# grant-froelich/Bathymetric-GNN

Measured on AMD Instinct MI355X. Metric: classified tile-nodes/s (fused graph build + 4-layer GAT forward + scatter), higher is better.
Workload: dtype f32

## Files before the change

### bathymetric-gnn_amd/csrc/bgnn_api.hip

```cpp
#include <stdarg.h>
#include <string.h>
#include <stdlib.h>

#include <algorithm>
#include <cmath>

#include "bgnn_internal.h"

namespace bgnn {

static thread_local char g_err[1024] = "";

void set_error(const char *fmt, ...) {
  va_list ap;
  va_start(ap, fmt);
  vsnprintf(g_err, sizeof(g_err), fmt, ap);
  va_end(ap);
}

int DevPool::alloc(size_t bytes, void **out) {
  if (bytes == 0) bytes = 256;
  bytes = (bytes + 255) & ~(size_t)255;
  auto it = free_blocks.lower_bound(bytes);
  if (it != free_blocks.end() && it->first <= bytes + bytes / 4 + 4096) {
// ... 177 lines not shown
}

using namespace bgnn;

extern "C" {

int bgnn_abi_version(void) { return BGNN_ABI_VERSION; }
const char *bgnn_last_error(void) { return g_err; }

int bgnn_ctx_create(int device, void *stream, bgnn_ctx **out) {
  BGNN_REQUIRE(out != nullptr, "bgnn_ctx_create: out is NULL");
  int n = 0;
  hipError_t e = hipGetDeviceCount(&n);
  if (e != hipSuccess || n <= 0) {
    (void)hipGetLastError();
    set_error("no HIP device available (%s)", e == hipSuccess ? "device count is 0" : hipGetErrorString(e));
    return BGNN_ERR_HIP;
  }
  BGNN_REQUIRE(device >= 0 && device < n, "bgnn_ctx_create: device %d out of range (have %d)", device, n);
  BGNN_HIP_CHECK(hipSetDevice(device));
  hipDeviceProp_t prop;
  BGNN_HIP_CHECK(hipGetDeviceProperties(&prop, device));
  bgnn_ctx *c = new bgnn_ctx();
  c->device = device;
  c->num_cus = prop.multiProcessorCount;
  if (stream) {
    c->stream = (hipStream_t)stream;
    c->owns_stream = false;
  } else {
    hipError_t se = hipStreamCreateWithFlags(&c->stream, hipStreamNonBlocking);
    if (se != hipSuccess) {
      delete c;
      set_error("hipStreamCreate failed: %s", hipGetErrorString(se));
      return BGNN_ERR_HIP;
    }
    c->owns_stream = true;
  }
  if (hipMalloc((void **)&c->zero_page, 16384) != hipSuccess || hipMemset(c->zero_page, 0, 16384) != hipSuccess) {
    set_error("zero page allocation failed");
    delete c;
    return BGNN_ERR_NOMEM;
  }
  c->stamps = reinterpret_cast<unsigned long long *>(c->zero_page + 1024);
  {
    auto env_int = [](const char *name, int dflt) { const char *e = getenv(name); return e ? atoi(e) : dflt; };
    BgnnOpts &o = c->opts;
    o.matrix_path = getenv("BGNN_BF16") ? 3 : getenv("BGNN_SPLIT_F16") ? 2 : getenv("BGNN_SPLIT_BF16") ? 1 : 0;
    o.fused = getenv("BGNN_NO_FUSED") ? 0 : 1;
    o.fold_extractor = getenv("BGNN_NO_FOLD") ? 0 : 1;
    o.ragged_atlas = getenv("BGNN_NO_ATLAS") ? 0 : 1;
    o.fused_front = getenv("BGNN_NO_FUSED_FRONT") ? 0 : 1;
    o.bf16_two_phase = getenv("BGNN_NO_TWO_PHASE") ? 0 : env_int("BGNN_TWO_PHASE", 1);
    o.bf16_layer0_af = getenv("BGNN_NO_LAYER0_AF") ? 0 : 1;
    o.stats_narrow = env_int("BGNN_STATS_NARROW", -1);
    o.diag_mask = env_int("BGNN_FUSED_DBG", 0);
    o.diag_stamps = getenv("BGNN_FUSED_STAMPS") ? 1 : 0;
    o.gemm_diag = env_int("BGNN_GEMM_DBG", 0);
    o.gemm_pair_major = getenv("BGNN_NO_PAIR_MAJOR") ? 0 : 1;
  }
  *out = c;
  return BGNN_OK;
}

static int *option_slot(bgnn_ctx *ctx, const char *name) {
  BgnnOpts &o = ctx->opts;
  struct { const char *n; int *p; } tab[] = {
      {"matrix_path", &o.matrix_path}, {"fused", &o.fused}, {"fold_extractor", &o.fold_extractor}, {"ragged_atlas", &o.ragged_atlas}, {"features_tiled", &o.features_tiled}, {"fused_front", &o.fused_front}, {"bf16_two_phase", &o.bf16_two_phase}, {"bf16_layer0_af", &o.bf16_layer0_af}, {"stats_narrow", &o.stats_narrow},
      {"diag_mask", &o.diag_mask}, {"diag_stamps", &o.diag_stamps}, {"gemm_diag", &o.gemm_diag}, {"gemm_pair_major", &o.gemm_pair_major}};
  for (auto &t : tab) if (strcmp(t.n, name) == 0) return t.p;
  return nullptr;
}

int bgnn_ctx_set_option(bgnn_ctx *ctx, const char *name, int value) {
  BGNN_REQUIRE(ctx && name, "bgnn_ctx_set_option: NULL argument");
  int *p = option_slot(ctx, name);
  BGNN_REQUIRE(p, "bgnn_ctx_set_option: unknown option '%s'", name);
  if (p == &ctx->opts.matrix_path) BGNN_REQUIRE(value >= 0 && value <= 3, "matrix_path=%d (0 exact f32, 1 bf16x3, 2 fp16x3, 3 bf16 storage)", value);
  if ((p == &ctx->opts.diag_mask || p == &ctx->opts.diag_stamps || p == &ctx->opts.gemm_diag) && value != 0)
    BGNN_REQUIRE(BGNN_DIAG, "option '%s' needs the diagnostic build of the library (python __graft_entry__.py --diag)", name);
  *p = value;
  return BGNN_OK;
}

int bgnn_ctx_get_option(bgnn_ctx *ctx, const char *name, int *value) {
  BGNN_REQUIRE(ctx && name && value, "bgnn_ctx_get_option: NULL argument");
  int *p = option_slot(ctx, name);
  BGNN_REQUIRE(p, "bgnn_ctx_get_option: unknown option '%s'", name);
  *value = *p;
  return BGNN_OK;
}

int bgnn_debug_stamps(bgnn_ctx *ctx, unsigned long long *out32) {
  if (!ctx || !out32) return BGNN_ERR_INVALID;
  (void)hipStreamSynchronize(ctx->stream);
  if (hipMemcpy(out32, ctx->stamps, 512, hipMemcpyDeviceToHost) != hipSuccess) return BGNN_ERR_HIP;
  (void)hipMemset(ctx->stamps, 0, 512);
  return BGNN_OK;
}

static void graph_free(bgnn_graph *g);

int bgnn_ctx_destroy(bgnn_ctx *ctx) {
  if (!ctx) return BGNN_OK;
  (void)hipSetDevice(ctx->device);
  (void)hipStreamSynchronize(ctx->stream);
  while (!ctx->live_graphs.empty()) graph_free(*ctx->live_graphs.begin());
  for (auto &r : ctx->prof_records) { (void)hipEventDestroy(r.start); (void)hipEventDestroy(r.stop); }
  for (auto &e : ctx->event_pool) (void)hipEventDestroy(e);
  for (auto &st : ctx->staging) { (void)hipEventDestroy(st.ev); (void)hipHostFree(st.p); }
  for (int i = 0; i < 7; ++i) if (ctx->ws[i]) (void)hipFree(ctx->ws[i]);
  for (auto &e : ctx->table_cache) { (void)hipFree(e.d_tiles); (void)hipFree(e.d_items); }
  if (ctx->zero_page) (void)hipFree(ctx->zero_page);
  ctx->pool.trim();
  for (auto &kv : ctx->pool.live) (void)hipFree(kv.first);
  if (ctx->owns_stream) (void)hipStreamDestroy(ctx->stream);
  delete ctx;
  return BGNN_OK;
}

int bgnn_ctx_synchronize(bgnn_ctx *ctx) {
// ... 585 lines not shown
```

### bathymetric-gnn_amd/csrc/bgnn_internal.h

```cpp
#pragma once
#include <hip/hip_runtime.h>
#include <stdint.h>
#include <stdio.h>
#include <string>
#include <cstdlib>
#include <vector>
#include <map>
#include <set>
#include <atomic>

#include "../../include/bgnn.h"
#include "../../include/bgnn_train.h"

namespace bgnn {

void set_error(const char *fmt, ...);

#define BGNN_HIP_CHECK(expr)                                                          \
  do {                                                                                \
    hipError_t _e = (expr);                                                           \
    if (_e != hipSuccess) {                                                           \
      bgnn::set_error("%s failed: %s (%s:%d)", #expr, hipGetErrorString(_e), __FILE__, \
                      __LINE__);                                                      \
      return BGNN_ERR_HIP;                                                            \
// ... 4 lines not shown
  do {                                 \
    if (!(cond)) {                     \
      bgnn::set_error(__VA_ARGS__);    \
      return BGNN_ERR_INVALID;         \
    }                                  \
  } while (0)

#define BGNN_TRY(expr)          \
  do {                          \
    int _r = (expr);            \
    if (_r != BGNN_OK) return _r; \
  } while (0)

struct DevPool {
  std::multimap<size_t, void *> free_blocks;
  std::map<void *, size_t> live;
  size_t total_bytes = 0;
  int alloc(size_t bytes, void **out);
  void release(void *p);
  void trim();
};

struct ProfRecord {
  int kernel;
  hipEvent_t start, stop;
};

struct WeightLayout {
  size_t fe_W0, fe_b0, fe_W1, fe_b1;
  struct Layer { size_t W, as, ad, ae, We, bias, bn_w, bn_b, bn_mean, bn_var, W2, b1; };
  std::vector<Layer> layers;
  size_t hd_W0[3], hd_b0[3], hd_W1[3], hd_b1[3];
  size_t total;
};

}

struct BgnnTileMeta {
  int32_t h, w;
  int32_t cell_off;
  int32_t pad;
  double rx, ry;
};

struct BgnnWorkItem {
  int32_t tile, r0, nr, pad;
};

struct BgnnOpts {
  int matrix_path = 0;
  int fused = 1;
  int fold_extractor = 1;
  int bf16_two_phase = 1;
  int bf16_layer0_af = 1;
  int stats_narrow = -1;
  int fused_front = 1;
  int features_tiled = 1;
  int ragged_atlas = 1;
  int diag_mask = 0;
  int diag_stamps = 0;
  int gemm_diag = 0;
  int gemm_pair_major = 1;
};

#ifndef BGNN_DIAG
#define BGNN_DIAG 0
#endif

struct bgnn_ctx {
  int device = 0;
  BgnnOpts opts;
  hipStream_t stream = nullptr;
  bool owns_stream = false;
  bgnn::DevPool pool;
  uint32_t prof_mask = 0;
  std::vector<bgnn::ProfRecord> prof_records;
  std::vector<hipEvent_t> event_pool;
  void *ws[7] = {nullptr, nullptr, nullptr, nullptr, nullptr, nullptr, nullptr};
  size_t ws_bytes[7] = {0, 0, 0, 0, 0, 0, 0};
  struct Staging { void *p; size_t cap; hipEvent_t ev; bool in_flight; };
  std::vector<Staging> staging;
  struct TableCache { int32_t n_tiles, h, w, item_cells; double rx, ry; BgnnTileMeta *d_tiles; BgnnWorkItem *d_items; int32_t n_items; uint64_t stamp; uint64_t id; int32_t refs; };
  std::vector<TableCache> table_cache;
  uint64_t table_stamp = 0, table_next_id = 1;
  std::set<struct bgnn_graph *> live_graphs;
  int num_cus = 256;
  float *zero_page = nullptr;
  unsigned long long *stamps = nullptr;
};

struct BgnnLayer {
  int d_in, heads, width;
  int concat;
  float *Wt;
  float *Wt_blk = nullptr;
  float *att_src;
  float *att_dst;
  float *V;
  float *scale;
  float *shift;
  float *Wsp;
  float *Wsp16;
  float Wsp16_inv = 1.0f;
  float *Wfp;
  float *Wbf;
  float *b1;
// ... 221 lines not shown
```

### bathymetric-gnn_amd/csrc/gat_layer_fused.hip

```cpp
#include <stdlib.h>
#include <algorithm>
#include <type_traits>
#include <utility>
#include "gat_tile_common.h"

namespace bgnn {

typedef float f32x16 __attribute__((ext_vector_type(16)));

enum { EPI_NEXT = 0, EPI_HEADS = 1 };

#if BGNN_DIAG
#define DBG(bit) (a.dbg & (bit))
#define BGNN_STAMP(slot)                                                                   \
  if (a.stamps) {                                                                          \
    const unsigned long long _t = __builtin_amdgcn_s_memtime();                            \
    t_sum[slot] += _t - t_prev;                                                            \
    t_prev = _t;                                                                           \
  }
#else
#define DBG(bit) false
#define BGNN_STAMP(slot)
#endif

// ... 1565 lines not shown
      constexpr int NC4 = NC * 4;
      const int t = 2 * cp + tt;
      const f32x16 &acc = tt ? acc1 : acc0;
      f32x4 s4[4], d4[4];
      s4[0] = lds_read4<0>(asl + t * 128); s4[1] = lds_read4<32>(asl + t * 128);
      s4[2] = lds_read4<64>(asl + t * 128); s4[3] = lds_read4<96>(asl + t * 128);
      d4[0] = lds_read4<NC4>(asl + t * 128); d4[1] = lds_read4<NC4 + 32>(asl + t * 128);
      d4[2] = lds_read4<NC4 + 64>(asl + t * 128); d4[3] = lds_read4<NC4 + 96>(asl + t * 128);
      lds_reads_done();
#pragma unroll
      for (int g = 0; g < 4; ++g) {
        const float4 v = make_float4(acc[4 * g], acc[4 * g + 1], acc[4 * g + 2], acc[4 * g + 3]);
        const f32x2 vlo = {v.x, v.y}, vhi = {v.z, v.w};
        ps_ += vlo * (f32x2){s4[g].x, s4[g].y}; ps_ += vhi * (f32x2){s4[g].z, s4[g].w};
        pd_ += vlo * (f32x2){d4[g].x, d4[g].y}; pd_ += vhi * (f32x2){d4[g].z, d4[g].w};
        typedef __bf16 bf16x4 __attribute__((ext_vector_type(4)));
        bf16x4 o;
        o[0] = (__bf16)v.x; o[1] = (__bf16)v.y; o[2] = (__bf16)v.z; o[3] = (__bf16)v.w;
        char *pb = patch + r * 128 + ((hl ^ ((r >> 3) & 1)) << 3);
        *reinterpret_cast<bf16x4 *>(pb + (((tt * 4 + g) ^ (r & 7)) << 4)) = o;
      }
      asm volatile("" : "+v"(ps_), "+v"(pd_));
      __builtin_amdgcn_sched_barrier(0);
    }
    sl_[cp] = ps_.x + ps_.y; dl_[cp] = pd_.x + pd_.y;
#pragma unroll
    for (int k = 0; k < NSTORE; ++k) {
      const int row = (lane >> 3) + 8 * k;
      uint4 q = *reinterpret_cast<const uint4 *>(patch + row * 128 + (((lane & 7) ^ (row & 7)) << 4));
      if (k & 1) q = make_uint4(q.z, q.w, q.x, q.y);
      char *prow = (rid_[k] >= 0 ? reinterpret_cast<char *>(a.out) + (int64_t)rid_[k] * (NC * 2) : reinterpret_cast<char *>(a.dump)) + (lane & 7) * 16;
      *reinterpret_cast<uint4 *>(prow + cp * 128) = q;
    }
    __builtin_amdgcn_sched_barrier(0);
  };
  col_pass(std::integral_constant<int, 0>{}); col_pass(std::integral_constant<int, 1>{});
  col_pass(std::integral_constant<int, 2>{}); col_pass(std::integral_constant<int, 3>{});
  {
    float srow[H2], drow_[H2];
#pragma unroll
    for (int hd = 0; hd < H2; ++hd) {
      const float sl = sl_[hd], dl = dl_[hd];
      srow[hd] = sl + __shfl_xor(sl, 32);
      drow_[hd] = dl + __shfl_xor(dl, 32);
    }
    if (id >= 0 && hl == 0) {
      float *ao = a.asd_out + (int64_t)id * 2 * H2;
      *reinterpret_cast<float4 *>(ao) = make_float4(srow[0], srow[1], srow[2], srow[3]);
      *reinterpret_cast<float4 *>(ao + 4) = make_float4(drow_[0], drow_[1], drow_[2], drow_[3]);
    }
  }
}

template <int K, bool AF = false>
static int launch_two_phase(bgnn_ctx *ctx, const FusedArgs &a) {
  constexpr size_t lds_bytes = (size_t)TwoPhaseLds<K>::BYTES;
  static std::atomic<uint64_t> configured{0};
  auto kern = gat_layer_bf16_2p_kernel<K, AF>;
  if (!(configured.load(std::memory_order_relaxed) >> (ctx->device & 63) & 1)) {
    BGNN_HIP_CHECK(hipFuncSetAttribute(reinterpret_cast<const void *>(kern), hipFuncAttributeMaxDynamicSharedMemorySize, (int)lds_bytes));
    configured.fetch_or(1ull << (ctx->device & 63), std::memory_order_relaxed);
  }
  hipLaunchKernelGGL(kern, dim3(a.tb.n_blocks), dim3(256), lds_bytes, ctx->stream, a);
  BGNN_HIP_CHECK(hipGetLastError());
  return BGNN_OK;
}

template <int HC, int C, int K, int NT, int EPI, int SP = 0, int AGG = 0>
static int launch_inst(bgnn_ctx *ctx, const FusedArgs &a) {
  constexpr size_t lds_bytes = (size_t)FusedLds<HC, C, K, NT, EPI, SP>::FLOATS * 4;
  static_assert(lds_bytes <= 160 * 1024, "one workgroup fits the CU's LDS");
  static std::atomic<uint64_t> configured{0};
  auto kern = gat_layer_fused_kernel<HC, C, K, NT, EPI, SP, AGG>;
  if (!(configured.load(std::memory_order_relaxed) >> (ctx->device & 63) & 1)) {
    BGNN_HIP_CHECK(hipFuncSetAttribute(reinterpret_cast<const void *>(kern), hipFuncAttributeMaxDynamicSharedMemorySize, (int)lds_bytes));
    configured.fetch_or(1ull << (ctx->device & 63), std::memory_order_relaxed);
  }
  hipLaunchKernelGGL(kern, dim3(a.tb.n_blocks), dim3(256), lds_bytes, ctx->stream, a);
  BGNN_HIP_CHECK(hipGetLastError());
  return BGNN_OK;
}

template <int HC, int NT, int EPI>
static int launch_by_stencil(bgnn_ctx *ctx, const bgnn_graph *g, int sp, const FusedArgs &a) {
  switch (sp) {
    case 0:
      return g->K == 8 ? launch_inst<HC, 64, 8, NT, EPI, 0>(ctx, a) : g->K == 4 ? launch_inst<HC, 64, 4, NT, EPI, 0>(ctx, a)
                                                                                 : launch_inst<HC, 64, 16, NT, EPI, 0>(ctx, a);
    case 3:
      return g->K == 8 ? launch_inst<HC, 64, 8, NT, EPI, 3>(ctx, a) : g->K == 4 ? launch_inst<HC, 64, 4, NT, EPI, 3>(ctx, a)
                                                                                 : launch_inst<HC, 64, 16, NT, EPI, 3>(ctx, a);
    default: break;
  }
  if (g->K == 16) return BGNN_ERR_UNSUPPORTED;
  if (sp == 1) return g->K == 8 ? launch_inst<HC, 64, 8, NT, EPI, 1>(ctx, a) : launch_inst<HC, 64, 4, NT, EPI, 1>(ctx, a);
  return g->K == 8 ? launch_inst<HC, 64, 8, NT, EPI, 2>(ctx, a) : launch_inst<HC, 64, 4, NT, EPI, 2>(ctx, a);
}

static bool fused_supported(const bgnn_graph *g, int C) {
  return g->kind == 0 && (g->K == 4 || g->K == 8 || g->K == 16) && g->n_blocks3 > 0 && C == 64 && g->max_w <= 8192 && g->compact_edges;
}

static void fill_common(FusedArgs &a, const bgnn_graph *g, const BgnnLayer &L, const float *V3, const void *xw, const float *asd, int relu) {
  a.tb.tiles = g->d_tiles; a.tb.items2 = g->uni_h ? nullptr : g->d_items3;
  a.tb.bh = g->bh3; a.tb.bw = g->bw3; a.tb.n_blocks = g->n_blocks3;
  a.node_id = g->d_node_id; a.cell_map = nullptr; a.tile_of_cell = nullptr;
  if (g->d_atlas) {
    a.tb.tiles = g->d_atlas_tile; a.tb.items2 = nullptr;
    a.tb.bh = g->atlas_h / 8; a.tb.bw = g->atlas_w / 16; a.tb.n_blocks = a.tb.bh * a.tb.bw;
    a.node_id = g->d_atlas; a.cell_map = g->d_cell_of_node; a.tile_of_cell = g->d_atlas_tile_of;
  }
  a.xw = xw; a.asd = asd; a.V = V3 ? V3 : L.V; a.scale = L.scale; a.shift = L.shift;
  a.slope = g->d_slope; a.node_depth = g->d_node_depth; a.tile_dist = g->d_tile_dist;
  a.relu = relu; a.zero_page = g->ctx->zero_page; a.dump = g->ctx->zero_page + 2048;
  a.dbg = BGNN_DIAG ? g->ctx->opts.diag_mask : 0;
  a.stamps = BGNN_DIAG && g->ctx->opts.diag_stamps ? g->ctx->stamps : nullptr;
}

int launch_fused_layer_next(bgnn_ctx *ctx, const bgnn_graph *g, const BgnnLayer &L, const BgnnLayer &Ln, int C, const float *V3,
                            const void *xw, const float *asd, void *xw_next, float *asd_next) {
  if (!fused_supported(g, C) || (!g->edge_default && !V3)) return BGNN_ERR_UNSUPPORTED;
  const int HC = L.heads * C, NC = Ln.heads * C;
  if (Ln.d_in != HC) return BGNN_ERR_UNSUPPORTED;
  FusedArgs a{};
  fill_common(a, g, L, V3, xw, asd, L.concat ? 1 : 0);
  int split = ctx->opts.matrix_path;
  if (split == 2 && !Ln.Wsp16) split = 1;
  a.Wt = split == 3 ? Ln.Wbf : split == 2 ? Ln.Wsp16 : split == 1 ? Ln.Wsp : Ln.Wfp;
  a.w_inv = Ln.Wsp16_inv;
  a.att_src = Ln.att_src; a.att_dst = Ln.att_dst; a.out = xw_next; a.asd_out = asd_next;
  a.H2 = Ln.heads; a.C2 = C;
  ProfScope ps(ctx, BGNN_K_FUSED);
  const bool main_shape = (HC == 256 && NC == 256) || (HC == 256 && NC == 64);
  if (split == 3 && !main_shape) return BGNN_ERR_UNSUPPORTED;
  if ((split == 1 || split == 2) && (!main_shape || g->K == 16)) { split = 0; a.Wt = Ln.Wfp; }
  if (split == 3 && HC == 256 && NC == 256 && C == 64 && ctx->opts.bf16_two_phase)
    return g->K == 8 ? launch_two_phase<8>(ctx, a) : g->K == 4 ? launch_two_phase<4>(ctx, a) : launch_two_phase<16>(ctx, a);
#define BGNN_FUSED_CASE(hc, nt) if (HC == hc && NC == nt * 32) return launch_by_stencil<hc, nt, EPI_NEXT>(ctx, g, split, a);
  BGNN_FUSED_CASE(256, 8) BGNN_FUSED_CASE(256, 2)
#undef BGNN_FUSED_CASE
  if (g->K == 16) return BGNN_ERR_UNSUPPORTED;
#define BGNN_FUSED_CASE(hc, nt)                                                                         \
  if (HC == hc && NC == nt * 32)                                                                        \
    return g->K == 8 ? launch_inst<hc, 64, 8, nt, EPI_NEXT>(ctx, a) : launch_inst<hc, 64, 4, nt, EPI_NEXT>(ctx, a);
  BGNN_FUSED_CASE(128, 4) BGNN_FUSED_CASE(128, 2) BGNN_FUSED_CASE(64, 2)
#undef BGNN_FUSED_CASE
  return BGNN_ERR_UNSUPPORTED;
}

int launch_fused_layer0_af(bgnn_ctx *ctx, const bgnn_graph *g, const BgnnLayer &L, const BgnnLayer &Ln, int C, const float *V3,
                           const void *h1, const float *asd, const float *W0af, const float *shift_af, void *xw_next, float *asd_next) {
  if (!fused_supported(g, C) || (!g->edge_default && !V3) || !W0af || !shift_af) return BGNN_ERR_UNSUPPORTED;
  if (C != 64 || L.heads != 4 || Ln.heads != 4 || Ln.d_in != 256 || !Ln.Wbf) return BGNN_ERR_UNSUPPORTED;
  FusedArgs a{};
  fill_common(a, g, L, V3, h1, asd, L.concat ? 1 : 0);
  a.shift = shift_af;
  a.Wt = Ln.Wbf; a.W0af = W0af;
  a.att_src = Ln.att_src; a.att_dst = Ln.att_dst; a.out = xw_next; a.asd_out = asd_next;
  a.H2 = Ln.heads; a.C2 = C;
  ProfScope ps(ctx, BGNN_K_FUSED);
  return g->K == 8 ? launch_two_phase<8, true>(ctx, a) : g->K == 4 ? launch_two_phase<4, true>(ctx, a) : launch_two_phase<16, true>(ctx, a);
}

int launch_fused_plain_layer(bgnn_ctx *ctx, const bgnn_graph *g, int mode, int C, const float *x, const float *dinv, const float *Wfp,
                             const float *ones, const float *post_scale, const float *post_shift, int post_relu, float *out) {
  if (!fused_supported(g, C) || !Wfp || mode < 1 || mode > 3) return BGNN_ERR_UNSUPPORTED;
  FusedArgs a{};
  BgnnLayer L{};
  L.V = nullptr; L.scale = const_cast<float *>(ones); L.shift = ctx->zero_page;
  fill_common(a, g, L, nullptr, x, dinv, 0);
  a.Wt = Wfp; a.att_src = post_scale; a.att_dst = post_shift; a.out = out; a.asd_out = nullptr;
  a.H2 = 1; a.C2 = C; a.relu2 = post_relu; a.self_loops = g->include_self_loops;
  ProfScope ps(ctx, BGNN_K_FUSED);
#define BGNN_PLAIN_CASE(M, HCV)                                                                                   \
  if (mode == M)                                                                                                  \
    return g->K == 8 ? launch_inst<HCV, 64, 8, 2, EPI_NEXT, 0, M>(ctx, a) : g->K == 4 ? launch_inst<HCV, 64, 4, 2, EPI_NEXT, 0, M>(ctx, a) \
                                                                                       : launch_inst<HCV, 64, 16, 2, EPI_NEXT, 0, M>(ctx, a);
  BGNN_PLAIN_CASE(1, 64) BGNN_PLAIN_CASE(2, 128) BGNN_PLAIN_CASE(3, 64)
#undef BGNN_PLAIN_CASE
  return BGNN_ERR_UNSUPPORTED;
}

bool fused_heads_available(const bgnn_ctx *ctx, const bgnn_graph *g, const bgnn_model *m) {
  if (!ctx->opts.fused || m->desc.gnn_type != BGNN_GNN_GAT || m->layers.empty()) return false;
  const BgnnLayer &L = m->layers.back();
  return fused_supported(g, m->desc.hidden) && L.heads == 1 && m->desc.num_classes <= 4 && m->head_hidden_total == 96 && m->hd_tab &&
         (m->desc.predict_correction ? 3 : 2) * (m->desc.hidden / 2) <= 96;
}

int launch_fused_layer_heads(bgnn_ctx *ctx, const bgnn_graph *g, const bgnn_model *m, const BgnnLayer &L, int C, const float *V3,
// ... 23 lines not shown
```

### bathymetric-gnn_amd/csrc/gat_tile_common.h

```cpp
#pragma once
#include "bgnn_internal.h"

namespace bgnn {

template <int K> struct StencilOffsets;
template <> struct StencilOffsets<4> {
  static constexpr int dr[4] = {-1, 1, 0, 0};
  static constexpr int dc[4] = {0, 0, -1, 1};
};
template <> struct StencilOffsets<8> {
  static constexpr int dr[8] = {-1, -1, -1, 0, 0, 1, 1, 1};
  static constexpr int dc[8] = {-1, 0, 1, -1, 1, -1, 0, 1};
};

template <> struct StencilOffsets<16> {
  static constexpr int dr[16] = {-1, -1, -1, 0, 0, 1, 1, 1, -2, -2, -2, 0, 0, 2, 2, 2};
  static constexpr int dc[16] = {-1, 0, 1, -1, 1, -1, 0, 1, -2, 0, 2, -2, 2, -2, 0, 2};
};

constexpr int TILE_W = 16;
constexpr int HALO_W = TILE_W + 2;
constexpr int TILED_PITCH = 36;
constexpr int TILE_H = 16, HALO_ROWS = (TILE_H + 2) * HALO_W;

template <int K>
__device__ __forceinline__ int slot_halo_offset(int b) {
  if (b >= K) return 0;
  if (K == 8) {
    const int k = b < 4 ? b : b + 1;
    return (k / 3 - 1) * (TILE_W + 2) + (k % 3 - 1);
  }
  return b == 0 ? -(TILE_W + 2) : b == 1 ? (TILE_W + 2) : b == 2 ? -1 : 1;
}

struct TileBlocks {
  const BgnnTileMeta *tiles;
  const BgnnWorkItem *items2;
  int bh, bw;
  int n_blocks;
};

struct BlockPos {
  int tile, r0, c0, h, w;
  int64_t cell_off;
};

template <int TH = TILE_H>
__device__ __forceinline__ BlockPos decode_block(const TileBlocks &tb) {
  const int bid = blockIdx.x, nb = tb.n_blocks;
  const int xcd = bid & 7, q = nb >> 3, r = nb & 7;
  const int wid = (xcd < r ? xcd * (q + 1) : r * (q + 1) + (xcd - r) * q) + (bid >> 3);
  BlockPos p;
  if (tb.items2) {
    const BgnnWorkItem it = tb.items2[wid];
    p.tile = it.tile; p.r0 = it.r0; p.c0 = it.nr;
  } else {
    const int bpt = tb.bh * tb.bw;
    p.tile = wid / bpt;
    const int rem = wid - p.tile * bpt;
    p.r0 = (rem / tb.bw) * TH; p.c0 = (rem % tb.bw) * TILE_W;
  }
  const BgnnTileMeta t = tb.tiles[p.tile];
  p.h = t.h; p.w = t.w; p.cell_off = t.cell_off;
  return p;
}

template <int H, int NTHREADS, int HROWS = HALO_ROWS>
__device__ __forceinline__ void load_halo_ids(const BlockPos &p, const int32_t *node_id, const float *asd, int *hid,
                                              float *has) {
  for (int idx = threadIdx.x; idx < HROWS; idx += NTHREADS) {
    const int gr = p.r0 + idx / HALO_W - 1, gc = p.c0 + idx % HALO_W - 1;
    int id = -1;
    if (gr >= 0 && gr < p.h && gc >= 0 && gc < p.w) {
      id = node_id[p.cell_off + (int64_t)gr * p.w + gc];
      if (id < 0) id = -1;
    }
    hid[idx] = id;
#pragma unroll
    for (int hh = 0; hh < H; ++hh) has[idx * H + hh] = id >= 0 ? asd[(int64_t)id * 2 * H + hh] : 0.0f;
  }
}

template <int H, int K, int H0, int NH>
__device__ __forceinline__ void attention_coefficients(int my, int self_idx, const int *hid, const float *has,
                                                       const float *asd, const float *eattr, const float *V, int ED,
                                                       float *out) {
  using Off = StencilOffsets<K>;
  float ea[K][4];
  float ea_sum[4] = {0.f, 0.f, 0.f, 0.f};
  int deg = 0;
  bool present[K];
  float eraw[K * 4];
  if (ED == 3 && (K * 3) % 4 == 0) {
    const float4 *ep = reinterpret_cast<const float4 *>(eattr + (int64_t)my * K * 3);
#pragma unroll
    for (int i = 0; i < K * 3 / 4; ++i) {
      const float4 v = ep[i];
      eraw[4 * i] = v.x; eraw[4 * i + 1] = v.y; eraw[4 * i + 2] = v.z; eraw[4 * i + 3] = v.w;
    }
  }
#pragma unroll
  for (int b = 0; b < K; ++b) {
    const int nidx = self_idx - Off::dr[b] * HALO_W - Off::dc[b];
    present[b] = hid[nidx] >= 0;
#pragma unroll
    for (int f = 0; f < 4; ++f) {
      float e = 0.0f;
      if (f < ED) e = (ED == 3 && (K * 3) % 4 == 0) ? eraw[(b * 3 + f) & (K * 4 - 1)] : eattr[((int64_t)my * K + b) * ED + f];
      ea[b][f] = (f < ED && present[b]) ? e : 0.0f;
      if (present[b]) ea_sum[f] += ea[b][f];
    }
    deg += present[b] ? 1 : 0;
  }
  const float cnt = (float)(deg > 0 ? deg : 1);
#pragma unroll
  for (int k = 0; k < NH; ++k) {
    const int hh = H0 + k;
// ... 221 lines not shown
```

### bathymetric-gnn_amd/runtime.py

```python
from __future__ import annotations

import ctypes as C
import os
import threading
from typing import Dict, Optional

import numpy as np
import torch

_PKG_DIR = os.path.dirname(os.path.abspath(__file__))
LIB_PATH = os.path.join(_PKG_DIR, "libbgnn_hip.so")

K_NAMES = ["scan", "stats", "features", "export", "gemm", "attcoef", "aggregate", "heads", "scatter", "fused"]
K_INDEX = {n: i for i, n in enumerate(K_NAMES)}

NODE_FEATURE_IDS = {"depth": 0, "local_mean": 1, "local_std": 2, "gradient_x": 3, "gradient_y": 4,
                    "gradient_magnitude": 5, "curvature": 6, "uncertainty": 7}
EDGE_FEATURE_IDS = {"distance": 0, "depth_difference": 1, "slope": 2}
EF_ZERO = 3

ERR_INVALID, ERR_HIP, ERR_NOMEM, ERR_UNSUPPORTED = -1, -2, -3, -4
ABI_VERSION = 7
MATRIX_PATHS = {"exact_f32": 0, "bf16x3": 1, "fp16x3": 2, "bf16": 3}
OPTION_NAMES = ("matrix_path", "fused", "fold_extractor", "ragged_atlas", "features_tiled", "fused_front",
                "bf16_two_phase", "bf16_layer0_af", "stats_narrow", "diag_mask", "diag_stamps",
                "gemm_diag", "gemm_pair_major")


GNN_TYPES = {"GAT": 0, "GCN": 1, "GraphSAGE": 2, "GIN": 3}


class ModelDesc(C.Structure):
    _fields_ = [("in_channels", C.c_int32), ("hidden", C.c_int32), ("num_layers", C.c_int32),
                ("heads", C.c_int32), ("num_classes", C.c_int32), ("edge_dim", C.c_int32),
                ("predict_correction", C.c_int32), ("bn_eps", C.c_float), ("gnn_type", C.c_int32)]


class Tiles(C.Structure):
    _fields_ = [("n_tiles", C.c_int32), ("hw", C.POINTER(C.c_int32)), ("resolution", C.POINTER(C.c_double)),
                ("depth", C.c_void_p), ("mask", C.c_void_p), ("uncertainty", C.c_void_p)]


class GraphOpts(C.Structure):
    _fields_ = [("connectivity", C.c_int32), ("include_self_loops", C.c_int32),
                ("n_node_features", C.c_int32), ("node_features", C.c_int32 * 8),
                ("n_edge_features", C.c_int32), ("edge_features", C.c_int32 * 4)]


class Outputs(C.Structure):
    _fields_ = [("class_logits", C.c_void_p), ("class_probs", C.c_void_p), ("predicted_class", C.c_void_p),
                ("confidence", C.c_void_p), ("correction", C.c_void_p), ("action", C.c_void_p),
                ("needs_review", C.c_void_p), ("auto_correct", C.c_void_p), ("hidden", C.c_void_p)]


class Dropout(C.Structure):
    _fields_ = [("p_extractor", C.c_float), ("p_attention", C.c_float), ("p_features", C.c_float), ("p_heads", C.c_float),
                ("seed", C.c_uint64)]


class OutputGrads(C.Structure):
    _fields_ = [("class_logits", C.c_void_p), ("class_probs", C.c_void_p), ("confidence", C.c_void_p), ("correction", C.c_void_p)]


_SIGNATURES = {
    "bgnn_abi_version": (C.c_int, []),
    "bgnn_last_error": (C.c_char_p, []),
    "bgnn_build_id": (C.c_char_p, []),
    "bgnn_ctx_create": (C.c_int, [C.c_int, C.c_void_p, C.POINTER(C.c_void_p)]),
    "bgnn_ctx_destroy": (C.c_int, [C.c_void_p]),
    "bgnn_ctx_synchronize": (C.c_int, [C.c_void_p]),
    "bgnn_ctx_stream": (C.c_void_p, [C.c_void_p]),
    "bgnn_ctx_set_option": (C.c_int, [C.c_void_p, C.c_char_p, C.c_int]),
    "bgnn_ctx_get_option": (C.c_int, [C.c_void_p, C.c_char_p, C.POINTER(C.c_int)]),
    "bgnn_ctx_profile": (C.c_int, [C.c_void_p, C.c_uint32]),
    "bgnn_ctx_profile_read": (C.c_int, [C.c_void_p, C.POINTER(C.c_double), C.POINTER(C.c_int64)]),
    "bgnn_model_weight_count": (C.c_size_t, [C.POINTER(ModelDesc)]),
    "bgnn_model_create": (C.c_int, [C.c_void_p, C.POINTER(ModelDesc), C.POINTER(C.c_float), C.c_size_t,
                                    C.POINTER(C.c_void_p)]),
# ... 314 lines not shown
```

Baseline: 308.1 million.

## Add persistent paired-block fused GAT layer kernel for exact f32 path

Adds a persistent 512-thread kernel in which two 256-thread halves each process their own tile block while sharing a double-buffered weight ring in LDS. The halves are offset by priority and barriers so one half stages the next weight chunk while the other runs gathers and MFMAs. Each block's epilogue is deferred into the next loop iteration so its stores overlap the next prologue. It is enabled by default for the f32 path with K=4 or 8 and no cell map, at the cost of one workgroup per CU and a large LDS footprint.

```diff
diff --git a/bathymetric-gnn_amd/csrc/bgnn_api.hip b/bathymetric-gnn_amd/csrc/bgnn_api.hip
--- a/bathymetric-gnn_amd/csrc/bgnn_api.hip
+++ b/bathymetric-gnn_amd/csrc/bgnn_api.hip
@@ -253,6 +253,7 @@
     o.fused_front = getenv("BGNN_NO_FUSED_FRONT") ? 0 : 1;
     o.bf16_two_phase = getenv("BGNN_NO_TWO_PHASE") ? 0 : env_int("BGNN_TWO_PHASE", 1);
     o.bf16_layer0_af = getenv("BGNN_NO_LAYER0_AF") ? 0 : 1;
+    o.fused_pair = getenv("BGNN_NO_FUSED_PAIR") ? 0 : 1;
     o.stats_narrow = env_int("BGNN_STATS_NARROW", -1);
     o.diag_mask = env_int("BGNN_FUSED_DBG", 0);
     o.diag_stamps = getenv("BGNN_FUSED_STAMPS") ? 1 : 0;
@@ -266,7 +267,7 @@
 static int *option_slot(bgnn_ctx *ctx, const char *name) {
   BgnnOpts &o = ctx->opts;
   struct { const char *n; int *p; } tab[] = {
-      {"matrix_path", &o.matrix_path}, {"fused", &o.fused}, {"fold_extractor", &o.fold_extractor}, {"ragged_atlas", &o.ragged_atlas}, {"features_tiled", &o.features_tiled}, {"fused_front", &o.fused_front}, {"bf16_two_phase", &o.bf16_two_phase}, {"bf16_layer0_af", &o.bf16_layer0_af}, {"stats_narrow", &o.stats_narrow},
+      {"matrix_path", &o.matrix_path}, {"fused", &o.fused}, {"fold_extractor", &o.fold_extractor}, {"ragged_atlas", &o.ragged_atlas}, {"features_tiled", &o.features_tiled}, {"fused_front", &o.fused_front}, {"bf16_two_phase", &o.bf16_two_phase}, {"bf16_layer0_af", &o.bf16_layer0_af}, {"fused_pair", &o.fused_pair}, {"stats_narrow", &o.stats_narrow},
       {"diag_mask", &o.diag_mask}, {"diag_stamps", &o.diag_stamps}, {"gemm_diag", &o.gemm_diag}, {"gemm_pair_major", &o.gemm_pair_major}};
   for (auto &t : tab) if (strcmp(t.n, name) == 0) return t.p;
   return nullptr;
diff --git a/bathymetric-gnn_amd/csrc/bgnn_internal.h b/bathymetric-gnn_amd/csrc/bgnn_internal.h
--- a/bathymetric-gnn_amd/csrc/bgnn_internal.h
+++ b/bathymetric-gnn_amd/csrc/bgnn_internal.h
@@ -80,6 +80,7 @@
   int fused = 1;
   int fold_extractor = 1;
   int bf16_two_phase = 1;
+  int fused_pair = 1;
   int bf16_layer0_af = 1;
   int stats_narrow = -1;
   int fused_front = 1;
diff --git a/bathymetric-gnn_amd/csrc/gat_layer_fused.hip b/bathymetric-gnn_amd/csrc/gat_layer_fused.hip
--- a/bathymetric-gnn_amd/csrc/gat_layer_fused.hip
+++ b/bathymetric-gnn_amd/csrc/gat_layer_fused.hip
@@ -1641,6 +1641,423 @@
   }
 }
 
+template <int K>
+struct PairLds {
+  static constexpr int HC = 256, NC = 256, H = 4, HR = FusedGeom<K>::HR;
+  static constexpr int WCHUNK = 32 * NC;
+  static constexpr int APITCH = (H * (K + 1)) | 1;
+  static constexpr int SLAB = HR * 32, ALPHA = 128 * APITCH;
+  static constexpr int SHARED = 2 * WCHUNK + 2 * HC + 2 * NC;
+  static constexpr int HALF = (SLAB + ALPHA + HR * (H + 1) + 2 * HR + 31) / 32 * 32;
+  static constexpr int BYTES = (SHARED + 2 * HALF) * 4;
+  static_assert(4 * 32 * TILED_PITCH <= SLAB, "the four store patches fit the half's own slab image");
+  static_assert(BYTES <= 160 * 1024, "one workgroup fits the CU's LDS");
+};
+
+template <int K>
+__global__ __launch_bounds__(512, 1) void gat_layer_pair_kernel(FusedArgs a, int n_pairs) {
+  constexpr int NTH = 256;
+  constexpr int HC = 256, C = 64, H = 4, NT = 8, NC = 256, NSLAB = HC / 32, SPH = C / 32;
+  using Geo = FusedGeom<K>;
+  using Lds = PairLds<K>;
+  using Off = StencilOffsets<K>;
+  constexpr int HR = Geo::HR, HW_ = Geo::HW, RAD = Geo::R;
+  constexpr int ROWB = 128, CPR = 8, APITCH = Lds::APITCH;
+  static_assert(K <= 8 && HR <= NTH, "one halo row per thread of a half");
+  extern __shared__ __attribute__((aligned(128))) float lds[];
+  const int tid_ = threadIdx.x & (NTH - 1), lane = threadIdx.x & 63;
+  const int tid = tid_;
+  const int wave8 = __builtin_amdgcn_readfirstlane(threadIdx.x >> 6);
+  const int half = wave8 >> 2, wave = wave8 & 3;
+  const int r = lane & 31, hl = lane >> 5;
+  const int cell = wave * 32 + r;
+  const int tr = cell / TILE_W, tc = cell % TILE_W;
+  const int self_idx = (tr + RAD) * HW_ + tc + RAD;
+  float *wring = lds;
+  float *scsh = wring + 2 * Lds::WCHUNK;
+  float *attr = scsh + 2 * HC;
+  float *slab = attr + 2 * NC + half * Lds::HALF;
+  float *alx = slab + Lds::SLAB;
+  float *has = alx + Lds::ALPHA;
+  float *hdp = has + H * HR;
+  int *hid2 = reinterpret_cast<int *>(hdp + HR);
+
+#if BGNN_DIAG
+  unsigned long long t_sum[12] = {0, 0, 0, 0, 0, 0, 0, 0, 0, 0, 0, 0};
+  unsigned long long t_prev = a.stamps ? __builtin_amdgcn_s_memtime() : 0;
+  const unsigned long long t_clk0 = t_prev, t_real0 = a.stamps ? __builtin_amdgcn_s_memrealtime() : 0;
+  unsigned long long n_blk = 0;
+#endif
+  auto stage_w_chunk = [&](int c) __attribute__((always_inline)) {
+    const char *src = reinterpret_cast<const char *>(a.Wt) + (uint32_t)(c * (Lds::WCHUNK * 4) + wave8 * 4096) + (uint32_t)(lane * 16);
+    float *dst = wring + (c & 1) * Lds::WCHUNK + wave8 * 1024;
+    const void *gs = reinterpret_cast<const void *>(src);
+    auto *ld = (__attribute__((address_space(3))) void *)dst;
+    __builtin_amdgcn_global_load_lds(gs, ld, 16, 0, 0);
+    __builtin_amdgcn_global_load_lds(gs, ld, 16, 1024, 0);
+    __builtin_amdgcn_global_load_lds(gs, ld, 16, 2048, 0);
+    __builtin_amdgcn_global_load_lds(gs, ld, 16, 3072, 0);
+  };
+  stage_w_chunk(0);
+  if (threadIdx.x < HC) {
+    const int c = threadIdx.x;
+    scsh[c] = a.scale[c]; scsh[HC + c] = a.shift[c];
+    attr[c] = a.att_src[c]; attr[NC + c] = a.att_dst[c];
+  }
+  wait_vm_lgkm<0>();
+  __builtin_amdgcn_s_barrier();
+  if (half) {
+    __builtin_amdgcn_s_setprio(1);
+    __builtin_amdgcn_s_barrier();
+  }
+
+  const uint32_t slab0 = lds_addr(slab);
+  const uint32_t wbuf0 = lds_addr(wring + 4 * hl * NC + r * WTileGroup<NT>::TG);
+  const uint32_t scsh0 = lds_addr(scsh) + hl * 16;
+  const uint32_t alx0 = lds_addr(alx + cell * APITCH);
+  constexpr uint32_t CX1 = 32, CX2 = 64, CX3 = 96;
+  constexpr int NHL = (H + 1) / 2;
+  constexpr int NPIECE = (HR * CPR + NTH - 1) / NTH;
+  static_assert(NTH % CPR == 0, "pieces advance by whole halo rows");
+  constexpr int RSTEP = NTH / CPR, RSTEP_R = RSTEP / HW_, RSTEP_C = RSTEP % HW_;
+  auto swz = [](int row) { return ((row % HW_) >> 1) & 7; };
+  static_assert(HW_ % 2 == 0 && NSLAB * ROWB <= 4096 && NSLAB % 2 == 0, "see gat_layer_fused_kernel; chunk 0 always lands in slot 0");
+
+  f32x16 acc[NT];
+  const char *dbase[NPIECE];
+  float eraw[K], adv[NHL], vpre[NHL][3];
+  float4 tdist;
+  f32x4 g[4];
+
+  auto issue_slab = [&](int s) __attribute__((always_inline)) {
+    const int sb = s * ROWB;
+#pragma unroll
+    for (int p = 0; p < NPIECE; ++p) {
+      if ((p + 1) * NTH <= HR * CPR || p * NTH + tid < HR * CPR) {
+        __builtin_amdgcn_global_load_lds(reinterpret_cast<const void *>(dbase[p] + sb),
+                                         (__attribute__((address_space(3))) void *)(slab + (p * NTH + wave * 64) * 4), 16, 0, 0);
+      }
+    }
+  };
+
+  auto prologue = [&](int blk, int *hid) __attribute__((always_inline)) {
+    const BlockPos pos = block_at<FT_H>(a.tb, blk);
+    const uint32_t cbase = (uint32_t)pos.cell_off, uw = (uint32_t)pos.w, uh = (uint32_t)pos.h;
+    const int h1 = pos.h - 1, w1 = pos.w - 1;
+    auto cell_index = [&](int gr, int gc) __attribute__((always_inline)) -> uint32_t {
+      const int r_ = max(0, min(gr, h1)), c_ = max(0, min(gc, w1));
+      return cbase + __umul24((uint32_t)r_, uw) + (uint32_t)c_;
+    };
+    auto node_at = [&](uint32_t cell_) __attribute__((always_inline)) -> int {
+      return *reinterpret_cast<const int *>(reinterpret_cast<const char *>(a.node_id) + (cell_ << 2));
+    };
+    auto in_tile = [&](int gr, int gc) __attribute__((always_inline)) -> bool { return (uint32_t)gr < uh && (uint32_t)gc < uw; };
+    int tid = tid_;
+    asm volatile("" : "+v"(tid));
+    const int cell_p = tid >> 6 << 5 | (tid & 31), hl = tid >> 5 & 1;
+    const int tr = cell_p / TILE_W, tc = cell_p % TILE_W;
+    const int hr_t = tid / HW_, hc_t = tid - hr_t * HW_;
+    const int gr_h = pos.r0 + hr_t - RAD, gc_h = pos.c0 + hc_t - RAD;
+    const int gr_m = pos.r0 + tr, gc_m = pos.c0 + tc;
+    const int raw_h = node_at(cell_index(gr_h, gc_h));
+    const int raw_m = node_at(cell_index(gr_m, gc_m));
+    int drow[NPIECE], prow_r[NPIECE], prow_c[NPIECE];
+    {
+      const int row0 = tid / CPR;
+      int pr = row0 / HW_, pc = row0 - pr * HW_;
+#pragma unroll
+      for (int p = 0; p < NPIECE; ++p) {
+        prow_r[p] = pr; prow_c[p] = pc;
+        drow[p] = node_at(cell_index(pos.r0 + pr - RAD, pos.c0 + pc - RAD));
+        pr += RSTEP_R; pc += RSTEP_C;
+        if (pc >= HW_) { pc -= HW_; pr += 1; }
+      }
+    }
+#pragma unroll
+    for (int i = 0; i < NHL; ++i)
+#pragma unroll
+      for (int f = 0; f < 3; ++f) vpre[i][f] = a.V[(hl + i * 2) * 3 + f];
+    const int hid_v = (tid < HR && in_tile(gr_h, gc_h) && raw_h >= 0) ? raw_h : -1;
+    const int my_pre = in_tile(gr_m, gc_m) ? raw_m : -1;
+#pragma unroll
+    for (int p = 0; p < NPIECE; ++p) {
+      const bool row_ok = (p + 1) * NTH <= HR * CPR || prow_r[p] < FT_H + 2 * RAD;
+      if (!(row_ok && in_tile(pos.r0 + prow_r[p] - RAD, pos.c0 + prow_c[p] - RAD))) drow[p] = -1;
+    }
+    float hasv[H];
+    const uint64_t hrow = (uint32_t)(hid_v >= 0 ? hid_v : 0), mrow = (uint32_t)(my_pre >= 0 ? my_pre : 0);
+    const float hdep = a.node_depth[hrow];
+    tdist = a.tile_dist[pos.tile];
+    {
+      const float4 v4 = *reinterpret_cast<const float4 *>(a.asd + hrow * 2 * H);
+      hasv[0] = v4.x; hasv[1] = v4.y; hasv[2] = v4.z; hasv[3] = v4.w;
+    }
+    const float4 *ep = reinterpret_cast<const float4 *>(a.slope + mrow * K);
+#pragma unroll
+    for (int i = 0; i < K / 4; ++i) {
+      const float4 q = ep[i];
+      eraw[4 * i] = q.x; eraw[4 * i + 1] = q.y; eraw[4 * i + 2] = q.z; eraw[4 * i + 3] = q.w;
+    }
+#pragma unroll
+    for (int i = 0; i < NHL; ++i) adv[i] = a.asd[mrow * 2 * H + H + hl + i * 2];
+    const char *xbase = reinterpret_cast<const char *>(a.xw);
+    const char *zp = reinterpret_cast<const char *>(a.zero_page);
+    {
+      const int cc = tid % CPR;
+#pragma unroll
+      for (int p = 0; p < NPIECE; ++p) {
+        const int row = prow_r[p] * HW_ + prow_c[p];
+        const int c = cc ^ swz(row);
+        dbase[p] = drow[p] >= 0 ? xbase + ((uint64_t)(uint32_t)drow[p] * (uint32_t)(HC * 4) + (uint32_t)(c * 16)) : zp;
+      }
+    }
+    if (tid < HR) {
+      hid[tid] = hid_v;
+#pragma unroll
+      for (int hh = 0; hh < H; ++hh) has[hh * HR + tid] = hid_v >= 0 ? hasv[hh] : -__builtin_inff();
+      hdp[tid] = hid_v >= 0 ? hdep : 0.0f;
+    }
+    {
+      float sink = tdist.x + tdist.y + tdist.z;
+#pragma unroll
+      for (int i = 0; i < NHL; ++i) sink += adv[i];
+#pragma unroll
+      for (int i = 0; i < K; ++i) sink += eraw[i];
+#pragma unroll
+      for (int i = 0; i < NHL; ++i) sink += vpre[i][0] + vpre[i][1] + vpre[i][2];
+      asm volatile("" ::"v"(sink));
+    }
+  };
+
+  auto phase_a = [&](const int *hid) __attribute__((always_inline)) {
+    const uint32_t hid0 = lds_addr(hid), has0 = lds_addr(has);
+    int lane_a = lane;
+    asm volatile("" : "+v"(lane_a));
+    const int hl_a = lane_a >> 5, cell_a = wave * 32 + (lane_a & 31);
+    const int self_a = (cell_a / TILE_W + RAD) * HW_ + cell_a % TILE_W + RAD;
+    const int my = lds_read1i<0>(hid0 + (uint32_t)self_a * 4u);
+    lds_reads_done();
+    float part[NHL][K + 1];
+    if (my < 0) {
+#pragma unroll
+      for (int i = 0; i < NHL; ++i)
+#pragma unroll
+        for (int b = 0; b <= K; ++b) part[i][b] = 0.0f;
+    } else {
+      using S = HaloSlot<K, HW_>;
+      int nb[K];
+      float hs[NHL][K + 1];
+      halo_ids<K, HW_>(hid0 + (uint32_t)(self_a - S::MAXOFF) * 4u, nb, std::make_integer_sequence<int, K>{});
+#pragma unroll
+      for (int i = 0; i < NHL; ++i)
+        halo_alpha_src<H, K, HW_>(has0 + (uint32_t)((hl_a + i * 2) * HR + self_a - S::MAXOFF) * 4u, hs[i], std::make_integer_sequence<int, K>{});
+      float dsrc[K + 1];
+      halo_depths<K, HW_>(lds_addr(hdp) + (uint32_t)(self_a - S::MAXOFF) * 4u, dsrc, std::make_integer_sequence<int, K>{});
+      lds_reads_done();
+      EdgeTerms<K> et;
+      edge_terms_compact<K>(nb, eraw, dsrc, tdist.x, tdist.y, tdist.z, et);
+      attention_head_pair<K, false>(et, hs[0], hs[1], adv[0], adv[1], vpre[0], vpre[1], part[0], part[1]);
+    }
+#pragma unroll
+    for (int i = 0; i < NHL; ++i)
+      lds_write_coefficients<K>(lds_addr(alx + cell_a * APITCH + (hl_a + i * 2) * (K + 1)), part[i], std::make_integer_sequence<int, K + 1>{});
+  };
+
+  auto gather = [&](int s) __attribute__((always_inline)) {
+    const uint32_t ap = alx0 + (s / SPH) * ((K + 1) * 4);
+#pragma unroll
+    for (int j = 0; j < 4; ++j) g[j] = (f32x4){0.f, 0.f, 0.f, 0.f};
+    auto nb_index = [&](int b) __attribute__((always_inline)) { return b >= K ? self_idx : self_idx - Off::dr[b < K ? b : 0] * HW_ - Off::dc[b < K ? b : 0]; };
+    f32x4 xb[2][4];
+    float al[2];
+    auto issue = [&](int b, int q) __attribute__((always_inline)) {
+      const int nidx = nb_index(b);
+      const int hcol = tc + RAD - (b < K ? Off::dc[b < K ? b : 0] : 0);
+      const uint32_t rb = slab0 + nidx * 128 + (((((hcol >> 1) & 7)) ^ hl) << 4);
+      al[q] = lds_read1<0>(ap + 4 * b);
+      xb[q][0] = lds_read4<0>(rb); xb[q][1] = lds_read4<0>(rb ^ CX1); xb[q][2] = lds_read4<0>(rb ^ CX2); xb[q][3] = lds_read4<0>(rb ^ CX3);
+    };
+    issue(0, 0);
+#pragma unroll
+    for (int b = 0; b <= K; ++b) {
+      const int q = b & 1;
+      if (b + 1 <= K) { issue(b + 1, q ^ 1); lds_reads_wait<5>(); } else lds_reads_done();
+#pragma unroll
+      for (int j = 0; j < 4; ++j) g[j] += al[q] * xb[q][j];
+    }
+    const uint32_t cp = scsh0 + s * 128;
+#pragma unroll
+    for (int jp = 0; jp < 2; ++jp) {
+      f32x4 sc0, sc1, sh0, sh1;
+      if (jp == 0) { sc0 = lds_read4<0>(cp); sc1 = lds_read4<CX1>(cp); sh0 = lds_read4<HC * 4>(cp); sh1 = lds_read4<HC * 4 + CX1>(cp); }
+      else { sc0 = lds_read4<CX2>(cp); sc1 = lds_read4<CX3>(cp); sh0 = lds_read4<HC * 4 + CX2>(cp); sh1 = lds_read4<HC * 4 + CX3>(cp); }
+      lds_reads_done();
+      g[2 * jp] = g[2 * jp] * sc0 + sh0;
+      g[2 * jp + 1] = g[2 * jp + 1] * sc1 + sh1;
+    }
+    if (a.relu) {
+#pragma unroll
+      for (int j = 0; j < 4; ++j) {
+        asm("v_max_f32 %0, 0, %0" : "+v"(g[j].x)); asm("v_max_f32 %0, 0, %0" : "+v"(g[j].y));
+        asm("v_max_f32 %0, 0, %0" : "+v"(g[j].z)); asm("v_max_f32 %0, 0, %0" : "+v"(g[j].w));
+      }
+    }
+  };
+
+  auto epilogue = [&](const int *hid) __attribute__((always_inline)) {
+    int lane_e = lane;
+    asm volatile("" : "+v"(lane_e));
+    const int r_e = lane_e & 31, hl_e = lane_e >> 5;
+    const int cell_e = wave * 32 + r_e;
+    const int id = hid[(cell_e / TILE_W + RAD) * HW_ + cell_e % TILE_W + RAD];
+    constexpr int TPH = C / 32, H2 = NT / TPH;
+    typedef float f32x2 __attribute__((ext_vector_type(2)));
+    f32x2 ps[H2], pd[H2];
+#pragma unroll
+    for (int hd = 0; hd < H2; ++hd) { ps[hd] = (f32x2){0.f, 0.f}; pd[hd] = (f32x2){0.f, 0.f}; }
+    const uint32_t asl = lds_addr(attr + 4 * hl_e);
+    float *patch = slab + wave * (32 * TILED_PITCH);
+    constexpr int LPR = 8, NSTORE = 32 * LPR / 64;
+    char *prow[NSTORE];
+#pragma unroll
+    for (int k = 0; k < NSTORE; ++k) {
+      const int c = wave * 32 + lane_e / LPR + (64 / LPR) * k;
+      const int rid = hid[(c / TILE_W + RAD) * HW_ + c % TILE_W + RAD];
+      prow[k] = (rid >= 0 ? reinterpret_cast<char *>(a.out) + (int64_t)rid * (NC * 4) : reinterpret_cast<char *>(a.dump)) + (lane_e % LPR) * 16;
+    }
+#pragma unroll
+    for (int t = 0; t < NT; ++t) {
+      f32x4 s4[4], d4[4];
+      s4[0] = lds_read4<0>(asl + t * 128); s4[1] = lds_read4<32>(asl + t * 128);
+      s4[2] = lds_read4<64>(asl + t * 128); s4[3] = lds_read4<96>(asl + t * 128);
+      d4[0] = lds_read4<NC * 4>(asl + t * 128); d4[1] = lds_read4<NC * 4 + 32>(asl + t * 128);
+      d4[2] = lds_read4<NC * 4 + 64>(asl + t * 128); d4[3] = lds_read4<NC * 4 + 96>(asl + t * 128);
+      lds_reads_done();
+#pragma unroll
+      for (int gq = 0; gq < 4; ++gq) {
+        const float4 v = make_float4(acc[t][4 * gq], acc[t][4 * gq + 1], acc[t][4 * gq + 2], acc[t][4 * gq + 3]);
+        const f32x2 vlo = {v.x, v.y}, vhi = {v.z, v.w};
+        ps[t / TPH] += vlo * (f32x2){s4[gq].x, s4[gq].y}; ps[t / TPH] += vhi * (f32x2){s4[gq].z, s4[gq].w};
+        pd[t / TPH] += vlo * (f32x2){d4[gq].x, d4[gq].y}; pd[t / TPH] += vhi * (f32x2){d4[gq].z, d4[gq].w};
+        *reinterpret_cast<float4 *>(patch + r_e * TILED_PITCH + 8 * gq + 4 * hl_e) = v;
+      }
+      asm volatile("" : "+v"(ps[t / TPH]), "+v"(pd[t / TPH]));
+      __builtin_amdgcn_sched_barrier(0);
+#pragma unroll
+      for (int k = 0; k < NSTORE; ++k)
+        *reinterpret_cast<float4 *>(prow[k] + t * 128) =
+            *reinterpret_cast<const float4 *>(patch + ((lane_e >> 3) + 8 * k) * TILED_PITCH + (lane_e & 7) * 4);
+      __builtin_amdgcn_sched_barrier(0);
+    }
+    float srow[H2], drow_[H2];
+#pragma unroll
+    for (int hd = 0; hd < H2; ++hd) {
+      const float sl = ps[hd].x + ps[hd].y, dl = pd[hd].x + pd[hd].y;
+      srow[hd] = sl + __shfl_xor(sl, 32);
+      drow_[hd] = dl + __shfl_xor(dl, 32);
+    }
+    if (id >= 0 && hl_e == 0) {
+      float *ao = a.asd_out + (int64_t)id * 2 * H2;
+      *reinterpret_cast<float4 *>(ao) = make_float4(srow[0], srow[1], srow[2], srow[3]);
+      *reinterpret_cast<float4 *>(ao + 4) = make_float4(drow_[0], drow_[1], drow_[2], drow_[3]);
+    }
+  };
+
+  auto slab_pair = [&](int s, auto first, auto work, bool last) __attribute__((always_inline)) {
+    constexpr bool WORK = decltype(work)::value;
+    const bool w_next = !(last && s + 1 == NSLAB);
+    if (half && w_next) stage_w_chunk((s + 1) & (NSLAB - 1));
+    if constexpr (WORK) gather(s);
+    __builtin_amdgcn_sched_barrier(0);
+    BGNN_STAMP(3)
+    wait_lgkm0();
+    __builtin_amdgcn_s_barrier();
+    __builtin_amdgcn_sched_barrier(0);
+    BGNN_STAMP(4)
+    if (!half && w_next) stage_w_chunk((s + 1) & (NSLAB - 1));
+    if constexpr (WORK) {
+      if (s + 1 < NSLAB) issue_slab(s + 1);
+      MfmaGroups<NT, NC, 0, 8, decltype(first)::value>::run(acc, g, wbuf0 + (uint32_t)(s & 1) * (Lds::WCHUNK * 4));
+    }
+    __builtin_amdgcn_sched_barrier(0);
+    BGNN_STAMP(5)
+    wait_vm_lgkm<0>();
+    __builtin_amdgcn_s_barrier();
+    __builtin_amdgcn_sched_barrier(0);
+    BGNN_STAMP(6)
+  };
+
+  const int G = gridDim.x;
+  bool prev_live = false;
+  int par = 0;
+#pragma unroll 1
+  for (int vp = blockIdx.x; vp < n_pairs; vp += G, par ^= 1) {
+    const bool last = vp + G >= n_pairs;
+    const int blk = 2 * xcd_order(vp, n_pairs) + half;
+    const bool live = blk < a.tb.n_blocks;
+    int *hid = hid2 + par * HR;
+    if (prev_live) epilogue(hid2 + (par ^ 1) * HR);
+    __builtin_amdgcn_sched_barrier(0);
+    BGNN_STAMP(0)
+    if (live) {
+      prologue(blk, hid);
+      BGNN_STAMP(1)
+      wait_vm_lgkm<0>();
+      __builtin_amdgcn_s_barrier();
+      __builtin_amdgcn_sched_barrier(0);
+      BGNN_STAMP(2)
+      issue_slab(0);
+      phase_a(hid);
+      BGNN_STAMP(7)
+      wait_vm_lgkm<0>();
+      __builtin_amdgcn_s_barrier();
+      BGNN_STAMP(8)
+      slab_pair(0, std::true_type{}, std::true_type{}, last);
+#pragma unroll 1
+      for (int s = 1; s < NSLAB; ++s) slab_pair(s, std::false_type{}, std::true_type{}, last);
+    } else {
+      wait_vm_lgkm<0>();
+      __builtin_amdgcn_s_barrier();
+      __builtin_amdgcn_s_barrier();
+#pragma unroll 1
+      for (int s = 0; s < NSLAB; ++s) slab_pair(s, std::false_type{}, std::false_type{}, last);
+    }
+    prev_live = live;
+#if BGNN_DIAG
+    n_blk += live ? 1 : 0;
+#endif
+  }
+  if (prev_live) epilogue(hid2 + (par ^ 1) * HR);
+  BGNN_STAMP(0)
+  if (!half) __builtin_amdgcn_s_barrier();
+#if BGNN_DIAG
+  if (a.stamps && lane == 0 && wave == 0) {
+    unsigned long long *own = a.stamps + 16;
+    for (int i = 0; i < 12; ++i) atomicAdd(own + i, t_sum[i]);
+    atomicAdd(own + 15, n_blk);
+    if (half == 0) {
+      atomicAdd(own + 13, __builtin_amdgcn_s_memtime() - t_clk0);
+      atomicAdd(own + 14, __builtin_amdgcn_s_memrealtime() - t_real0);
+    }
+  }
+#endif
+}
+
+template <int K>
+static int launch_pair(bgnn_ctx *ctx, const FusedArgs &a) {
+  constexpr size_t lds_bytes = (size_t)PairLds<K>::BYTES;
+  static std::atomic<uint64_t> configured{0};
+  auto kern = gat_layer_pair_kernel<K>;
+  if (!(configured.load(std::memory_order_relaxed) >> (ctx->device & 63) & 1)) {
+    BGNN_HIP_CHECK(hipFuncSetAttribute(reinterpret_cast<const void *>(kern), hipFuncAttributeMaxDynamicSharedMemorySize, (int)lds_bytes));
+    configured.fetch_or(1ull << (ctx->device & 63), std::memory_order_relaxed);
+  }
+  const int n_pairs = (a.tb.n_blocks + 1) / 2;
+  hipLaunchKernelGGL(kern, dim3(std::min(n_pairs, ctx->num_cus)), dim3(512), lds_bytes, ctx->stream, a, n_pairs);
+  BGNN_HIP_CHECK(hipGetLastError());
+  return BGNN_OK;
+}
+
 template <int K, bool AF = false>
 static int launch_two_phase(bgnn_ctx *ctx, const FusedArgs &a) {
   constexpr size_t lds_bytes = (size_t)TwoPhaseLds<K>::BYTES;
@@ -1725,6 +2142,8 @@
   if ((split == 1 || split == 2) && (!main_shape || g->K == 16)) { split = 0; a.Wt = Ln.Wfp; }
   if (split == 3 && HC == 256 && NC == 256 && C == 64 && ctx->opts.bf16_two_phase)
     return g->K == 8 ? launch_two_phase<8>(ctx, a) : g->K == 4 ? launch_two_phase<4>(ctx, a) : launch_two_phase<16>(ctx, a);
+  if (split == 0 && HC == 256 && NC == 256 && C == 64 && a.cell_map == nullptr && ctx->opts.fused_pair && (g->K == 8 || g->K == 4))
+    return g->K == 8 ? launch_pair<8>(ctx, a) : launch_pair<4>(ctx, a);
 #define BGNN_FUSED_CASE(hc, nt) if (HC == hc && NC == nt * 32) return launch_by_stencil<hc, nt, EPI_NEXT>(ctx, g, split, a);
   BGNN_FUSED_CASE(256, 8) BGNN_FUSED_CASE(256, 2)
 #undef BGNN_FUSED_CASE
diff --git a/bathymetric-gnn_amd/csrc/gat_tile_common.h b/bathymetric-gnn_amd/csrc/gat_tile_common.h
--- a/bathymetric-gnn_amd/csrc/gat_tile_common.h
+++ b/bathymetric-gnn_amd/csrc/gat_tile_common.h
@@ -45,11 +45,12 @@
   int64_t cell_off;
 };
 
+__device__ __forceinline__ int xcd_order(int bid, int nb) {
+  const int xcd = bid & 7, q = nb >> 3, r = nb & 7;
+  return (xcd < r ? xcd * (q + 1) : r * (q + 1) + (xcd - r) * q) + (bid >> 3);
+}
 template <int TH = TILE_H>
-__device__ __forceinline__ BlockPos decode_block(const TileBlocks &tb) {
-  const int bid = blockIdx.x, nb = tb.n_blocks;
-  const int xcd = bid & 7, q = nb >> 3, r = nb & 7;
-  const int wid = (xcd < r ? xcd * (q + 1) : r * (q + 1) + (xcd - r) * q) + (bid >> 3);
+__device__ __forceinline__ BlockPos block_at(const TileBlocks &tb, int wid) {
   BlockPos p;
   if (tb.items2) {
     const BgnnWorkItem it = tb.items2[wid];
@@ -63,6 +64,10 @@
   const BgnnTileMeta t = tb.tiles[p.tile];
   p.h = t.h; p.w = t.w; p.cell_off = t.cell_off;
   return p;
+}
+template <int TH = TILE_H>
+__device__ __forceinline__ BlockPos decode_block(const TileBlocks &tb) {
+  return block_at<TH>(tb, xcd_order(blockIdx.x, tb.n_blocks));
 }
 
 template <int H, int NTHREADS, int HROWS = HALO_ROWS>
diff --git a/bathymetric-gnn_amd/runtime.py b/bathymetric-gnn_amd/runtime.py
--- a/bathymetric-gnn_amd/runtime.py
+++ b/bathymetric-gnn_amd/runtime.py
@@ -23,7 +23,7 @@
 ABI_VERSION = 7
 MATRIX_PATHS = {"exact_f32": 0, "bf16x3": 1, "fp16x3": 2, "bf16": 3}
 OPTION_NAMES = ("matrix_path", "fused", "fold_extractor", "ragged_atlas", "features_tiled", "fused_front",
-                "bf16_two_phase", "bf16_layer0_af", "stats_narrow", "diag_mask", "diag_stamps",
+                "bf16_two_phase", "bf16_layer0_af", "fused_pair", "stats_narrow", "diag_mask", "diag_stamps",
                 "gemm_diag", "gemm_pair_major")
 
 
```

After: 299.5 million. 2.8% lower.
